# XuyangBai/PointDSC

Hardware: AMD Instinct MI355X
Metric: point-cloud pairs/sec @ N=5000 corr (higher is better)
Workload: dtype f32 (attention products as fp16x3 split (fp16 hi+lo operand pairs, three f16 MFMAs per product), f32 accumulate; fc_message / PointCN products as fp16 hi+lo split; spatial-consistency matrix stored as unorm16); 1 GPU; 3DMatch-like synthetic correspondences (BASELINE.json configs[2]): N=5000 corr, 32 pairs per step sharded over 1 GPU(s) = 32 per GPU, 12-layer PointDSC, seeded random weights; num_corr=5000, pairs_per_gpu=32, global_batch=32, compat_format=u16, layer_gemm=h3, att_leaves=canonical, latency_mode=False, range_guard=lazy (pipeline), collective=none (single process, no process group)

## Files before the change

include/pointdsc_hip.h:

```cpp
#ifndef POINTDSC_HIP_H
#define POINTDSC_HIP_H

#include <stddef.h>

#ifdef __cplusplus
extern "C" {
#endif

#define PDSC_VERSION 9
#define PDSC_CHANNELS 128
#define PDSC_MAX_K 64
#define PDSC_MAX_POWER_ITERS 32

enum pdsc_status {
    PDSC_OK = 0,
    PDSC_ERR_ARG = -1,
    PDSC_ERR_WORKSPACE = -2,
    PDSC_ERR_LAUNCH = -3
};

typedef struct pdsc_config {
    int in_dim;
    int num_layers;
    int num_channels;
// ... 128 lines not shown
size_t pdsc_wfrag_fold_head_bytes(void);
int pdsc_layer_prefers_block(int bs, int N);
int pdsc_layer_h3_uses_coop(int bs, int N);
size_t pdsc_wfrag_tail_bytes(void);
size_t pdsc_wfrag_head_bytes(void);
int pdsc_wfrag_build_tail(const float* w1, const float* b1, const float* w2, const float* b2, const float* w3,
                          const float* b3, void* out, int gemm_format, void* stream);
int pdsc_wfrag_build_head(const float* wp, const float* bp, const float* wq, const float* bq, void* out,
                          int gemm_format, void* stream);

size_t pdsc_attention_scratch_bytes(int bs, int N, int nsplit);
int    pdsc_attention_default_split(int bs, int N);
int    pdsc_sc_attention(const float* qkv, const float* compat, long long ld, float* msg,
                         void* scratch, size_t scratch_bytes, int bs, int N, int nsplit, void* stream);

size_t pdsc_split_q_bytes(int bs, int N);
size_t pdsc_split_kv_bytes(int bs, int N);
int    pdsc_pack_qkv_split(const float* qkv, void* q_split, void* kv_tiles, int bs, int N, void* stream);
size_t pdsc_attention_split_scratch_bytes(int bs, int N, int nsplit);
int    pdsc_attention_split_default_split(int bs, int N);
int    pdsc_attention_leaf_count(int N);
int    pdsc_attention_leaf_plan(int bs, int N, int leaves_mode, int* nsplit, int* nleaf);
size_t pdsc_attention_leaf_scratch_bytes(int bs, int N, int leaves_mode);
int    pdsc_sc_attention_split(const void* q_split, const void* kv_tiles, const float* compat, long long ld,
                               float* msg, void* scratch, size_t scratch_bytes, int bs, int N, int nsplit,
                               void* stream);
int    pdsc_sc_attention_split_u16(const void* q_split, const void* kv_tiles, const unsigned short* compat_u16, long long ld,
                                   float* msg, void* scratch, size_t scratch_bytes, int bs, int N, int nsplit,
                                   void* stream);

int pdsc_attention_trace(long long* device_buffer);

int pdsc_attention_leaf_split_override(int d);

int pdsc_layer_trace(long long* device_buffer);

int pdsc_classifier_hidden(const float* feat, const float* W1, const float* b1, const float* W2, const float* b2, float* h2,
                           int M, void* stream);

int pdsc_normalize_confidence(const float* feat, const float* h2, const float* w3, const float* b3,
                              float* normed, float* conf, int M, void* stream);

int pdsc_nms_keys(const float* src_keypts, const float* conf, float radius, float* keys,
                  int bs, int N, void* stream);
size_t pdsc_nms_workspace_bytes(int bs, int N);
int pdsc_nms_keys_grid(const float* src_keypts, const float* conf, float radius, float* keys, void* workspace,
                       size_t workspace_bytes, int bs, int N, void* stream);
int pdsc_rank_select(const float* keys, int* seeds, int bs, int N, int num_seeds, void* stream);

int pdsc_knn_seeds(const float* normed, const int* seeds, float* dist_scratch, int* knn_idx,
                   int bs, int N, int S, int k, void* stream);
int pdsc_knn_seeds_form(const float* normed, const float* normed_pf, const int* seeds, float* dist_scratch, int* knn_idx,
                        int bs, int N, int S, int k, int form, void* stream);
int pdsc_normalize_confidence_pf(const float* feat, const float* h2, const float* w3, const float* b3, float* normed,
                                 float* normed_pf, float* conf, int bs, int N, void* stream);

int pdsc_seed_power_iteration(const float* normed, const float* src_keypts, const float* tgt_keypts,
                              const int* knn_idx, const float* sigma, const float* sigma_spat,
                              float* eig_iters, unsigned int* conv_mask, float* seed_M,
                              int bs, int N, int S, int k, int num_iterations, void* stream);

int pdsc_seed_transforms(const float* src_keypts, const float* tgt_keypts, const int* knn_idx,
                         const float* eig_iters, const unsigned int* conv_mask, float* seed_trans,
                         float* seed_weights ,
                         int bs, int N, int S, int k, int num_iterations, void* stream);

int pdsc_seed_solve(const float* normed, const float* src_keypts, const float* tgt_keypts, const int* knn_idx,
                    const float* sigma, const float* sigma_spat, float* eig_iters, unsigned int* conv_mask, float* seed_M,
                    float* seed_trans, float* seed_weights, int bs, int N, int S, int k, int num_iterations, void* stream);

int pdsc_rigid_transform_3d(const float* A, const float* B, const float* weights, float weight_threshold,
                            float* T, int bs, int n, void* stream);

int pdsc_score_hypotheses(const float* seed_trans, const float* src_keypts, const float* tgt_keypts,
                          float inlier_threshold, int* counts, int bs, int N, int S, void* stream);
int pdsc_select_best(const int* counts, const float* seed_trans, const float* src_keypts,
                     const float* tgt_keypts, float inlier_threshold, int* best, float* initial_trans,
                     float* labels, int bs, int N, int S, void* stream);

int pdsc_post_refinement(const float* initial_trans, const float* src_keypts, const float* tgt_keypts,
                         float threshold, int max_iters, float* final_trans, int* solves,
                         int bs, int N, void* stream);

int pdsc_forward_testing(const pdsc_config* cfg, const float* wpack, const void* wsplit ,
                         const float* corr_pos, const float* src_keypts, const float* tgt_keypts,
                         int bs, int N, int num_seeds,
                         float* final_trans, float* final_labels,
                         void* workspace, size_t workspace_bytes, void* stream);

int pdsc_forward_testing_ragged(const pdsc_config* cfg, const float* wpack, const void* wsplit,
                                const float* corr_pos, const float* src_keypts, const float* tgt_keypts,
                                int bs, int N, int num_seeds, const int* num_corr, const int* num_seeds_per_pair, int n_min,
                                float* final_trans, float* final_labels,
                                void* workspace, size_t workspace_bytes, void* stream);

int pdsc_forward_testing_streams(const pdsc_config* cfg, const float* wpack, const void* wsplit,
                                 const float* corr_pos, const float* src_keypts, const float* tgt_keypts,
                                 int bs, int N, int num_seeds, const int* num_corr ,
                                 const int* num_seeds_per_pair, int n_min,
                                 float* final_trans, float* final_labels,
                                 void* workspace, size_t workspace_bytes,
                                 void* stream, void* tail_stream, void* fork_event, void* join_event);

int pdsc_forward_validation(const pdsc_config* cfg, const float* wpack, const void* wsplit,
                            const float* corr_pos, const float* src_keypts, const float* tgt_keypts,
                            int bs, int N, int num_seeds, float* final_trans, float* logits,
// ... 155 lines not shown
```

pointdsc_amd/_lib.py:

```python
from __future__ import annotations

import ctypes as C
import os
from pathlib import Path

PKG = Path(__file__).resolve().parent
LIB_PATH = Path(os.environ.get("POINTDSC_HIP_LIB", PKG / "libpointdsc_hip.so"))


class PointDSCLibraryError(RuntimeError):
    pass


class PdscConfig(C.Structure):
    _fields_ = [
        ("in_dim", C.c_int), ("num_layers", C.c_int), ("num_channels", C.c_int),
        ("num_iterations", C.c_int), ("k", C.c_int), ("refine_iters", C.c_int),
        ("inlier_threshold", C.c_float), ("nms_radius", C.c_float), ("refine_threshold", C.c_float),
        ("attention_precision", C.c_int), ("compat_format", C.c_int), ("layer_gemm", C.c_int),
        ("att_leaves", C.c_int), ("value_fold", C.c_int),
    ]


W_SECTIONS = [
# ... 16 lines not shown
SIGNATURES = {
    "pdsc_version": (_i, []),
    "pdsc_set_range_report": (_i, [_vp]),
    "pdsc_last_error": (C.c_char_p, []),
    "pdsc_experiments_enabled": (_i, []),
    "pdsc_wpack_floats": (_ll, [_cfgp]),
    "pdsc_wpack_offset": (_ll, [_cfgp, _i, _i]),
    "pdsc_compat_ld": (_ll, [_i]),
    "pdsc_workspace_bytes": (_sz, [_cfgp, _i, _i, _i]),
    "pdsc_workspace_offset": (_ll, [_cfgp, _i, _i, _i, C.c_char_p]),
    "pdsc_spatial_compat": (_i, [_vp, _vp, _vp, _vp, _vp, _ll, _i, _i, _vp]),
    "pdsc_spatial_compat_u16": (_i, [_vp, _vp, _vp, _vp, _ll, _i, _i, _vp]),
    "pdsc_selftest_exact_math": (_i, [_vp, _f, _vp, _vp, _ll, _vp]),
    "pdsc_selftest_mfma_valu_neighbour": (_i, [_vp, _i, _i, _vp]),
    "pdsc_classifier_hidden": (_i, [_vp, _vp, _vp, _vp, _vp, _vp, _i, _vp]),
    "pdsc_linear": (_i, [_vp, _ll, _vp, _vp, _vp, _ll, _vp, _ll, _i, _i, _i, _i, _vp]),
    "pdsc_layer0": (_i, [_vp, _i, _vp, _vp, _vp, _i, _vp]),
    "pdsc_layer_run": (_i, [C.POINTER(PdscLayerCall), _vp]),
    "pdsc_wsplit_bytes": (_sz, [_cfgp]),
    "pdsc_wsplit_offset": (_ll, [_cfgp, _i, _i]),
    "pdsc_wsplit_build": (_i, [_cfgp, _vp, _vp, _vp]),
    "pdsc_layer_prefers_block": (_i, [_i, _i]),
    "pdsc_layer_h3_uses_coop": (_i, [_i, _i]),
    "pdsc_wfrag_tail_bytes": (_sz, []),
    "pdsc_wfrag_head_bytes": (_sz, []),
    "pdsc_wfrag_fold_tail_bytes": (_sz, []),
    "pdsc_wfrag_fold_head_bytes": (_sz, []),
    "pdsc_wfrag_build_tail": (_i, [_vp] * 7 + [_i, _vp]),
    "pdsc_wfrag_build_head": (_i, [_vp] * 5 + [_i, _vp]),
    "pdsc_sc_attention_split_partials": (_i, [_vp, _vp, _vp, _i, _ll, _vp, _sz, _i, _i, _i, _i, _vp]),
    "pdsc_split_q_bytes": (_sz, [_i, _i]),
    "pdsc_split_kv_bytes": (_sz, [_i, _i]),
    "pdsc_pack_qkv_split": (_i, [_vp, _vp, _vp, _i, _i, _vp]),
    "pdsc_attention_split_scratch_bytes": (_sz, [_i, _i, _i]),
    "pdsc_attention_split_default_split": (_i, [_i, _i]),
    "pdsc_attention_leaf_count": (_i, [_i]),
    "pdsc_attention_leaf_plan": (_i, [_i, _i, _i, C.POINTER(C.c_int), C.POINTER(C.c_int)]),
    "pdsc_attention_leaf_scratch_bytes": (_sz, [_i, _i, _i]),
    "pdsc_attention_trace": (_i, [_vp]),
    "pdsc_attention_leaf_split_override": (_i, [_i]),
    "pdsc_layer_trace": (_i, [_vp]),
    "pdsc_sc_attention_split": (_i, [_vp, _vp, _vp, _ll, _vp, _vp, _sz, _i, _i, _i, _vp]),
    "pdsc_sc_attention_split_u16": (_i, [_vp, _vp, _vp, _ll, _vp, _vp, _sz, _i, _i, _i, _vp]),
    "pdsc_attention_scratch_bytes": (_sz, [_i, _i, _i]),
    "pdsc_attention_default_split": (_i, [_i, _i]),
    "pdsc_sc_attention": (_i, [_vp, _vp, _ll, _vp, _vp, _sz, _i, _i, _i, _vp]),
    "pdsc_normalize_confidence": (_i, [_vp, _vp, _vp, _vp, _vp, _vp, _i, _vp]),
    "pdsc_nms_keys": (_i, [_vp, _vp, _f, _vp, _i, _i, _vp]),
    "pdsc_nms_workspace_bytes": (_sz, [_i, _i]),
    "pdsc_nms_keys_grid": (_i, [_vp, _vp, _f, _vp, _vp, _sz, _i, _i, _vp]),
    "pdsc_rank_select": (_i, [_vp, _vp, _i, _i, _i, _vp]),
    "pdsc_knn_seeds": (_i, [_vp, _vp, _vp, _vp, _i, _i, _i, _i, _vp]),
    "pdsc_knn_seeds_form": (_i, [_vp, _vp, _vp, _vp, _vp, _i, _i, _i, _i, _i, _vp]),
    "pdsc_normalize_confidence_pf": (_i, [_vp, _vp, _vp, _vp, _vp, _vp, _vp, _i, _i, _vp]),
    "pdsc_seed_power_iteration": (_i, [_vp, _vp, _vp, _vp, _vp, _vp, _vp, _vp, _vp, _i, _i, _i, _i, _i, _vp]),
    "pdsc_seed_solve": (_i, [_vp] * 11 + [_i, _i, _i, _i, _i, _vp]),
    "pdsc_seed_transforms": (_i, [_vp, _vp, _vp, _vp, _vp, _vp, _vp, _i, _i, _i, _i, _i, _vp]),
    "pdsc_rigid_transform_3d": (_i, [_vp, _vp, _vp, _f, _vp, _i, _i, _vp]),
    "pdsc_score_hypotheses": (_i, [_vp, _vp, _vp, _f, _vp, _i, _i, _i, _vp]),
    "pdsc_select_best": (_i, [_vp, _vp, _vp, _vp, _f, _vp, _vp, _vp, _i, _i, _i, _vp]),
    "pdsc_post_refinement": (_i, [_vp, _vp, _vp, _f, _i, _vp, _vp, _i, _i, _vp]),
    "pdsc_profile_enable": (_i, [_i]),
    "pdsc_profile_reset": (_i, []),
    "pdsc_profile_set_stride": (_i, [_i, _i]),
    "pdsc_profile_read": (_i, [_i, C.POINTER(C.c_double), C.POINTER(C.c_int)]),
    "pdsc_match_scratch_bytes": (_sz, [_i, _i]),
    "pdsc_match_descriptors": (_i, [_vp, _vp, _i, _i, _i, _vp, _vp, _vp, _sz, _vp]),
    "pdsc_match_descriptors_ip": (_i, [_vp, _vp, _i, _i, _i, _vp, _vp, _vp, _sz, _vp]),
    "pdsc_select_correspondences": (_i, [_vp, _vp, _i, _vp, _vp, _vp]),
    "pdsc_build_corr_pos": (_i, [_vp, _vp, _vp, _vp, _vp, _vp, _vp, _vp]),
    "pdsc_sm_workspace_bytes": (_sz, [_i, _i]),
    "pdsc_sm_baseline": (_i, [_vp, _vp, _vp, _f, _i, _i, _vp, _vp, _vp, _vp, _sz, _i, _i, _vp]),
    "pdsc_sm_baseline_form": (_i, [_vp, _vp, _vp, _f, _i, _i, _vp, _vp, _vp, _vp, _sz, _i, _i, _i, _vp]),
    "pdsc_pmc_adjacency": (_i, [_vp, _f, _vp, _ll, _i, _i, _vp]),
    "pdsc_pmc_workspace_bytes": (_sz, [_i, _i]),
    "pdsc_pmc_baseline": (_i, [_vp, _vp, _vp, _f, _i, _vp, _vp, _vp, _vp, _vp, _sz, _i, _i, _vp]),
    "pdsc_pmc_baseline_ex": (_i, [_vp, _vp, _vp, _f, _i, _vp, _vp, _vp, _vp, _vp, _sz, _i, _i, _i, C.POINTER(C.c_float), _vp]),
    "pdsc_cal_confidence_workspace_bytes": (_sz, [_i, _i]),
    "pdsc_cal_confidence": (_i, [_vp, _ll, _vp, _i, _i, _vp, _vp, _sz, _i, _i, _vp]),
    "pdsc_eval_stats": (_i, [_vp, _vp, _vp, _vp, _f, _f, _vp, _i, _i, _vp]),
    "pdsc_loss_workspace_bytes": (_sz, [_i, _i]),
    "pdsc_classification_loss": (_i, [_vp, _vp, _vp, _i, _vp, _vp, _vp, _sz, _i, _i, _vp]),
    "pdsc_sm_loss_matrix": (_i, [_vp, _ll, _vp, _i, _vp, _vp, _vp, _sz, _i, _i, _vp]),
    "pdsc_sm_loss_features": (_i, [_vp, _vp, _vp, _i, _vp, _vp, _vp, _vp, _sz, _i, _i, _vp]),
    "pdsc_transformation_loss": (_i, [_vp, _vp, _vp, _vp, _vp, _f, _f, _vp, _vp, _sz, _i, _i, _vp]),
    "pdsc_sc_attention_lse": (_i, [_vp, _vp, _ll, _vp, _vp, _vp, _sz, _i, _i, _i, _vp]),
    "pdsc_attention_backward_workspace_bytes": (_sz, [_i, _i]),
    "pdsc_sc_attention_backward": (_i, [_vp, _vp, _ll, _vp, _vp, _vp, _vp, _vp, _sz, _i, _i, _vp]),
    "pdsc_attention_backward_default_split": (_i, [_i, _i]),
    "pdsc_attention_backward_split_workspace_bytes": (_sz, [_i, _i, _i]),
    "pdsc_sc_attention_backward_split": (_i, [_vp, _vp, _ll, _vp, _vp, _vp, _vp, _vp, _sz, _i, _i, _i, _vp]),
    "pdsc_feature_compat_backward_workspace_bytes": (_sz, [_i, _i]),
    "pdsc_feature_compat_backward": (_i, [_vp, _vp, _vp, _ll, _vp, _vp, _vp, _sz, _i, _i, _vp]),
    "pdsc_seed_solve_backward_workspace_bytes": (_sz, [_i, _i, _i, _i]),
    "pdsc_seed_solve_backward": (_i, [_vp] * 11 + [_sz, _i, _i, _i, _i, _i, _vp]),
    "pdsc_transformation_loss_grad": (_i, [_vp, _vp, _vp, _vp, _vp, _vp, _sz, _i, _i, _vp]),
    "pdsc_icp_workspace_bytes": (_sz, [_i, _i, _i]),
    "pdsc_icp_refine": (_i, [_vp, _vp, _vp, _vp, _vp, C.c_double, C.c_double, C.c_double, _i, _vp, _vp, _vp, _vp, _vp, _vp, _vp,
                             _sz, _i, _i, _i, _vp]),
    "pdsc_information_workspace_bytes": (_sz, [_i, _i, _i]),
    "pdsc_information_matrix": (_i, [_vp, _vp, _vp, _vp, _vp, C.c_double, _vp, _vp, _vp, _vp, _sz, _i, _i, _i, _vp]),
    "pdsc_voxel_keys": (_i, [_vp, _vp, C.c_double, _vp, _i, _i, _vp]),
    "pdsc_voxel_means": (_i, [_vp, _vp, _vp, _vp, _vp, _i, _i, _vp]),
    "pdsc_hybrid_neighbours_workspace_bytes": (_sz, [_i, _i]),
    "pdsc_hybrid_neighbours": (_i, [_vp, _vp, C.c_double, _i, _vp, _vp, _vp, _vp, _sz, _i, _i, _vp]),
    "pdsc_estimate_normals": (_i, [_vp, _vp, _vp, _vp, _i, C.POINTER(C.c_double), _vp, _i, _i, _vp]),
# ... 57 lines not shown
```

pointdsc_amd/csrc/seeds.hip:

```cpp
#include <math.h>
#include <stdlib.h>
#include "pdsc_common.h"
#include "ragged.h"

namespace pdsc {

int knn_dist_rows(const float* normed, const int* seeds, float* dist, long long ldd, int bs, int N, int S,
                  hipStream_t st);

__global__ __launch_bounds__(256) void normalize_conf_kernel(const float* __restrict__ feat, const float* __restrict__ h2,
                                                             const float* __restrict__ w3, const float* __restrict__ b3,
                                                             float* __restrict__ normed, float* __restrict__ conf, int M) {
    const int lane = threadIdx.x & 63;
    const long long row = (long long)blockIdx.x * 4 + (threadIdx.x >> 6);
    if (row >= M) return;
    const float2 v = *reinterpret_cast<const float2*>(feat + row * PDSC_CHANNELS + lane * 2);
    const float ss = wave_sum(fmaf(v.y, v.y, v.x * v.x));
    const float nrm = fmaxf(sqrtf(ss), 1e-12f);
    float2 o;
    o.x = v.x / nrm;
    o.y = v.y / nrm;
    *reinterpret_cast<float2*>(normed + row * PDSC_CHANNELS + lane * 2) = o;
    float p = lane < 32 ? h2[row * 32 + lane] * w3[lane] : 0.f;
    p = wave_sum(p);
// ... 464 lines not shown
        if (splits < min_splits) splits = min_splits;
        if (splits > N) splits = N;
        const int slice = pdsc::ceil_div(N, splits);
        splits = pdsc::ceil_div(N, slice);
        hipLaunchKernelGGL(pdsc::nms_flags_kernel, dim3(row_blocks, splits, bs), dim3(256), 0, st, src, conf, radius2, keys, N, slice);
        return pdsc::check_launch("pdsc_nms_keys");
    }
}

static float nms_radius2(float radius) { return pdsc::sqrt_threshold_radicand(radius); }

extern "C" size_t pdsc_nms_workspace_bytes(int bs, int N) {
    if (bs <= 0 || N <= 0) return 0;
    return (size_t)bs * pdsc::nms_ws_pair_bytes(N);
}

namespace pdsc {

int launch_nms_keys_grid(const float* src, const float* conf, float radius, float* keys, void* workspace, size_t workspace_bytes,
                         int bs, int N, const int* nvalid, hipStream_t st) {
    PDSC_REQUIRE(src && conf && keys, "pdsc_nms_keys_grid: null pointer");
    PDSC_REQUIRE(bs > 0 && N > 0, "pdsc_nms_keys_grid: bs=%d N=%d", bs, N);
    if (!(radius > 0.f) || !(radius < INFINITY) || !workspace) {
        PDSC_REQUIRE(!nvalid, "pdsc_nms_keys_grid: ragged batches need a positive finite nms_radius and the grid workspace");
        return pdsc_nms_keys(src, conf, radius, keys, bs, N, st);
    }
    if (workspace_bytes < pdsc_nms_workspace_bytes(bs, N)) {
        set_error("pdsc_nms_keys_grid: workspace %zu < %zu bytes", workspace_bytes, pdsc_nms_workspace_bytes(bs, N));
        return PDSC_ERR_WORKSPACE;
    }
    const size_t ws_pair = nms_ws_pair_bytes(N);
    hipLaunchKernelGGL(nms_grid_kernel, dim3(bs), dim3(1024), 0, st, src, conf, radius, (unsigned char*)workspace, ws_pair, N, nvalid);
    int rc = check_launch("pdsc_nms_keys_grid(grid)");
    if (rc != PDSC_OK) return rc;
    hipLaunchKernelGGL(nms_window_kernel, dim3(ceil_div(N, 256), bs), dim3(256), 0, st, (const unsigned char*)workspace, ws_pair,
                       nms_radius2(radius), keys, N, nvalid);
    return check_launch("pdsc_nms_keys_grid(window)");
}

int launch_rank_select(const float* keys, int* seeds, int bs, int N, int num_seeds, const int* nvalid, const int* svalid, hipStream_t st,
                       unsigned int* conv_mask_init) {
    PDSC_REQUIRE(keys && seeds, "pdsc_rank_select: null pointer");
    PDSC_REQUIRE(bs > 0 && N > 0 && num_seeds >= 0 && num_seeds <= N, "pdsc_rank_select: bs=%d N=%d S=%d", bs, N, num_seeds);
    if (num_seeds == 0) return conv_mask_init ? launch_fill_u32(conv_mask_init, 0xFFFFFFFFu, (size_t)bs, st) : PDSC_OK;
    const size_t lds_bytes = (size_t)num_seeds * sizeof(unsigned long long);
    PDSC_REQUIRE(lds_bytes <= 128 * 1024, "pdsc_rank_select: num_seeds=%d exceeds the single-workgroup LDS list (16384)", num_seeds);
    const int rc = ensure_dynamic_lds(reinterpret_cast<const void*>(&seed_select_kernel), lds_bytes > 65536 ? 128 * 1024 : 65536,
                                      "pdsc_rank_select(dynamic LDS)");
    if (rc != PDSC_OK) return rc;
    hipLaunchKernelGGL(seed_select_kernel, dim3(bs), dim3(SEL_THREADS), lds_bytes, st, keys, seeds, N, num_seeds, nvalid, svalid, conv_mask_init);
    return check_launch("pdsc_rank_select");
}

constexpr int KF_ROWS = 32, KF_CAP = 256, KF_KEEP = 96, KF_MAX_WANT = 48;

struct KnnFusedArgs {
    const float* X;
    const float* Xpf;
    const int* seeds;
    int* knn_idx;
    int NS, S, k, idx_bits;
    int bs, nrb;
    const int* nvalid;
};

__global__ __launch_bounds__(256, 2) void knn_fused_kernel(KnnFusedArgs a) {
    extern __shared__ __attribute__((aligned(16))) unsigned long long kf_dyn[];
    unsigned long long (*list)[KF_CAP] = reinterpret_cast<unsigned long long (*)[KF_CAP]>(kf_dyn);
    __shared__ float tau[KF_ROWS];
    __shared__ int cnt[KF_ROWS];
    __shared__ unsigned long long gmin[4][64];
    const int t = threadIdx.x, lane = t & 63, wave = t >> 6, l31 = lane & 31, h = lane >> 5;
    int b, rb;
    {
        const int nrb = a.nrb, L = blockIdx.x;
        if ((a.bs & 7) == 0) {
            const int xcd = L & 7, idx = L >> 3;
            b = xcd + 8 * (idx / nrb);
            rb = idx % nrb;
        } else {
            b = L / nrb;
            rb = L % nrb;
        }
    }
    const int r0 = rb * KF_ROWS;
    const int N = a.nvalid ? a.nvalid[b] : a.NS;
    const float* X = a.X + (size_t)b * a.NS * PDSC_CHANNELS;
    const int want = a.k + 1;
    const unsigned long long idx_mask = (1ULL << a.idx_bits) - 1ULL;
    if (t < KF_ROWS) { tau[t] = INFINITY; cnt[t] = 0; }

    f32x4 af[16];
    {
        const int row = a.seeds[(size_t)b * a.S + min(r0 + l31, a.S - 1)];
        const float* p = X + (size_t)row * PDSC_CHANNELS + 4 * h;
#pragma unroll
        for (int q = 0; q < 16; ++q) af[q] = *reinterpret_cast<const f32x4*>(p + 8 * q);
    }
    const int nblocks = (N + 31) >> 5, rounds = (nblocks + 3) >> 2;
    f32x4 bf[16];
    const int Npf = (a.NS + 31) & ~31;
    const float* Xpf = a.Xpf ? a.Xpf + (size_t)b * Npf * PDSC_CHANNELS + lane * 4 : nullptr;
    auto load_b = [&](int cb) {
        if (Xpf) {
            const float* p = Xpf + (size_t)min(cb, nblocks - 1) * 32 * PDSC_CHANNELS;
#pragma unroll
            for (int q = 0; q < 16; ++q) bf[q] = *reinterpret_cast<const f32x4*>(p + 256 * q);
        } else {
            const int col = min(cb * 32 + l31, N - 1);
            const float* p = X + (size_t)col * PDSC_CHANNELS + 4 * h;
#pragma unroll
            for (int q = 0; q < 16; ++q) bf[q] = *reinterpret_cast<const f32x4*>(p + 8 * q);
        }
    };
    load_b(wave);
    __syncthreads();
    for (int rd = 0; rd < rounds; ++rd) {
        const int cb = rd * 4 + wave;
        f32x16 acc;
#pragma unroll
        for (int r = 0; r < 16; ++r) acc[r] = 0.f;
#pragma unroll
        for (int q = 0; q < 16; ++q)
#pragma unroll
            for (int e = 0; e < 4; ++e) acc = __builtin_amdgcn_mfma_f32_32x32x2f32(af[q][e], bf[q][e], acc, 0, 0, 0);
        load_b(cb + 4);
        const int col = cb * 32 + l31;
        if (col < N) {
#pragma unroll
            for (int r = 0; r < 16; ++r) {
                const int row = (r & 3) + 8 * (r >> 2) + 4 * h;
                const float v = 2.0f - 2.0f * acc[r];
                if (v <= tau[row] && r0 + row < a.S) {
                    const unsigned long long key = ((unsigned long long)float_order_bits(v) << a.idx_bits) | (unsigned)col;
                    const int slot = atomicAdd(&cnt[row], 1);
                    list[row][slot] = key;
                }
            }
        }
        __syncthreads();
        for (int rr = 0; rr < 8; ++rr) {
            const int row = wave * 8 + rr;
            const int n = cnt[row];
            if (n <= KF_CAP - 128) continue;
            unsigned long long e[KF_CAP / 64], mine = ~0ULL;
#pragma unroll
            for (int u = 0; u < KF_CAP / 64; ++u) {
                e[u] = lane + 64 * u < n ? list[row][lane + 64 * u] : ~0ULL;
                mine = e[u] < mine ? e[u] : mine;
            }
            gmin[wave][lane] = mine;
            __builtin_amdgcn_fence(__ATOMIC_RELEASE, "wavefront");
            __builtin_amdgcn_wave_barrier();
            __builtin_amdgcn_fence(__ATOMIC_ACQUIRE, "wavefront");
            int rk = 0;
#pragma unroll 8
            for (int u = 0; u < 64; ++u) rk += gmin[wave][u] < mine;
            const unsigned long long vote = __ballot(rk == want - 1);
            const int src = __ffsll((long long)vote) - 1;
            unsigned long long ub = ((unsigned long long)(unsigned)__builtin_amdgcn_readlane((int)(mine >> 32), src) << 32) |
                                    (unsigned)__builtin_amdgcn_readlane((int)(mine & 0xffffffffULL), src);
            int kept = 0;
#pragma unroll
            for (int u = 0; u < KF_CAP / 64; ++u) {
                const bool keep = e[u] <= ub;
                const unsigned long long bal = __ballot(keep);
                if (keep) list[row][kept + __popcll(bal & ((1ULL << lane) - 1ULL))] = e[u];
                kept += __popcll(bal);
            }
            __builtin_amdgcn_fence(__ATOMIC_RELEASE, "wavefront");
            __builtin_amdgcn_wave_barrier();
            __builtin_amdgcn_fence(__ATOMIC_ACQUIRE, "wavefront");
            if (kept > KF_KEEP) {
                unsigned long long f[KF_CAP / 64], cand = 0ULL;
                int rank[KF_CAP / 64];
#pragma unroll
                for (int u = 0; u < KF_CAP / 64; ++u) { f[u] = lane + 64 * u < kept ? list[row][lane + 64 * u] : ~0ULL; rank[u] = 0; }
                for (int j = 0; j < kept; ++j) {
                    const unsigned long long o = list[row][j];
#pragma unroll
                    for (int u = 0; u < KF_CAP / 64; ++u) rank[u] += o < f[u];
                }
                __builtin_amdgcn_fence(__ATOMIC_RELEASE, "wavefront");
                __builtin_amdgcn_wave_barrier();
                __builtin_amdgcn_fence(__ATOMIC_ACQUIRE, "wavefront");
#pragma unroll
                for (int u = 0; u < KF_CAP / 64; ++u) {
                    const bool real = lane + 64 * u < kept;
                    if (real && rank[u] < want) list[row][rank[u]] = f[u];
                    if (real && rank[u] == want - 1) cand = f[u];
                }
                const unsigned long long who = __ballot(cand != 0ULL);
                const int sl = __ffsll((long long)who) - 1;
                ub = ((unsigned long long)(unsigned)__builtin_amdgcn_readlane((int)(cand >> 32), sl) << 32) |
                     (unsigned)__builtin_amdgcn_readlane((int)(cand & 0xffffffffULL), sl);
                kept = want;
            }
            if (lane == 0) {
                cnt[row] = kept;
                const unsigned int ob = (unsigned int)(ub >> a.idx_bits);
                tau[row] = __uint_as_float((ob & 0x80000000u) ? (ob & 0x7fffffffu) : ~ob);
            }
        }
        __syncthreads();
    }
    for (int rr = 0; rr < 8; ++rr) {
        const int row = wave * 8 + rr;
        if (r0 + row >= a.S) continue;
        const int n = cnt[row];
        unsigned long long f[KF_CAP / 64];
        int rank[KF_CAP / 64];
#pragma unroll
        for (int u = 0; u < KF_CAP / 64; ++u) { f[u] = lane + 64 * u < n ? list[row][lane + 64 * u] : ~0ULL; rank[u] = 0; }
        for (int j = 0; j < n; ++j) {
            const unsigned long long o = list[row][j];
#pragma unroll
            for (int u = 0; u < KF_CAP / 64; ++u) rank[u] += o < f[u];
        }
#pragma unroll
        for (int u = 0; u < KF_CAP / 64; ++u)
            if (lane + 64 * u < n && rank[u] >= 1 && rank[u] < want)
                a.knn_idx[((size_t)b * a.S + r0 + row) * a.k + (rank[u] - 1)] = (int)(f[u] & idx_mask);
    }
}

int launch_knn_seeds(const float* normed, const int* seeds, float* dist_scratch, int* knn_idx, int bs, int N, int S, int k,
                     const int* nvalid, hipStream_t st) {
    return launch_knn_seeds_form(normed, nullptr, seeds, dist_scratch, knn_idx, bs, N, S, k, nvalid, 0, st);
}

bool knn_seeds_uses_fused(int bs, int N, int S, int k) {
    return k + 1 <= KF_MAX_WANT && N >= 256 && (long long)bs * ceil_div(S, KF_ROWS) >= 384;
}

int launch_knn_seeds_form(const float* normed, const float* normed_pf, const int* seeds, float* dist_scratch, int* knn_idx, int bs, int N,
                          int S, int k, const int* nvalid, int form, hipStream_t st) {
    PDSC_REQUIRE(form >= 0 && form <= 2, "pdsc_knn_seeds: form=%d", form);
    const bool fits = k + 1 <= KF_MAX_WANT && N >= 256;
    PDSC_REQUIRE(form != 2 || fits, "pdsc_knn_seeds: the fused form needs k + 1 <= %d and N >= 256 (k=%d, N=%d)", KF_MAX_WANT, k, N);
    if (form == 2 || (form == 0 && knn_seeds_uses_fused(bs, N, S, k))) {
        PDSC_REQUIRE(normed && seeds && knn_idx, "pdsc_knn_seeds: null pointer");
        PDSC_REQUIRE(bs > 0 && N > 1 && S > 0, "pdsc_knn_seeds: bs=%d N=%d S=%d", bs, N, S);
        PDSC_REQUIRE(k >= 1 && k <= PDSC_MAX_K && k <= N - 1, "pdsc_knn_seeds: k=%d (N=%d, max %d)", k, N, PDSC_MAX_K);
        KnnFusedArgs a{};
        a.X = normed; a.Xpf = normed_pf; a.seeds = seeds; a.knn_idx = knn_idx; a.NS = N; a.S = S; a.k = k; a.nvalid = nvalid;
        a.idx_bits = 1;
        while ((1 << a.idx_bits) < N) ++a.idx_bits;
        const size_t lds_bytes = (size_t)KF_ROWS * KF_CAP * sizeof(unsigned long long);
        const int rc_lds = ensure_dynamic_lds(reinterpret_cast<const void*>(&knn_fused_kernel), lds_bytes, "pdsc_knn_seeds(fused, dynamic LDS)");
        if (rc_lds != PDSC_OK) return rc_lds;
        a.bs = bs; a.nrb = ceil_div(S, KF_ROWS);
        hipLaunchKernelGGL(knn_fused_kernel, dim3((unsigned)(a.nrb * bs)), dim3(256), lds_bytes, st, a);
        return check_launch("pdsc_knn_seeds(fused)");
    }

    PDSC_REQUIRE(normed && seeds && dist_scratch && knn_idx, "pdsc_knn_seeds: null pointer");
    PDSC_REQUIRE(bs > 0 && N > 1 && S > 0, "pdsc_knn_seeds: bs=%d N=%d S=%d", bs, N, S);
    PDSC_REQUIRE(k >= 1 && k <= PDSC_MAX_K && k <= N - 1, "pdsc_knn_seeds: k=%d (N=%d, max %d)", k, N, PDSC_MAX_K);
    PDSC_REQUIRE((size_t)N * 4 <= 144 * 1024, "pdsc_knn_seeds: N=%d exceeds the single-workgroup LDS row (36864)", N);
    const long long ldd = pdsc_compat_ld(N);
    int rc = knn_dist_rows(normed, seeds, dist_scratch, ldd, bs, N, S, st);
    if (rc != PDSC_OK) return rc;
    int idx_bits = 1;
    while ((1 << idx_bits) < N) ++idx_bits;
    const size_t lds_bytes = (size_t)N * sizeof(unsigned int);
    {
        const int rc_lds = ensure_dynamic_lds(reinterpret_cast<const void*>(&knn_select_kernel), 144 * 1024, "pdsc_knn_seeds(dynamic LDS)");
        if (rc_lds != PDSC_OK) return rc_lds;
    }
    hipLaunchKernelGGL(knn_select_kernel, dim3(S, bs), dim3(KNN_THREADS), lds_bytes, st, dist_scratch, ldd, knn_idx, N, S, k, idx_bits, nvalid);
    return check_launch("pdsc_knn_seeds");
}

}

extern "C" int pdsc_nms_keys_grid(const float* src, const float* conf, float radius, float* keys, void* workspace,
                                  size_t workspace_bytes, int bs, int N, void* stream) {
    return pdsc::launch_nms_keys_grid(src, conf, radius, keys, workspace, workspace_bytes, bs, N, nullptr, (hipStream_t)stream);
}

extern "C" int pdsc_rank_select(const float* keys, int* seeds, int bs, int N, int num_seeds, void* stream) {
    return pdsc::launch_rank_select(keys, seeds, bs, N, num_seeds, nullptr, nullptr, (hipStream_t)stream);
}

extern "C" int pdsc_knn_seeds_form(const float* normed, const float* normed_pf, const int* seeds, float* dist_scratch, int* knn_idx,
                                   int bs, int N, int S, int k, int form, void* stream) {
    return pdsc::launch_knn_seeds_form(normed, normed_pf, seeds, dist_scratch, knn_idx, bs, N, S, k, nullptr, form, (hipStream_t)stream);
}

extern "C" int pdsc_normalize_confidence_pf(const float* feat, const float* h2, const float* w3, const float* b3, float* normed,
                                            float* normed_pf, float* conf, int bs, int N, void* stream) {
    return pdsc::launch_normalize_conf_pf(feat, h2, w3, b3, normed, normed_pf, conf, bs, N, (hipStream_t)stream);
}

extern "C" int pdsc_knn_seeds(const float* normed, const int* seeds, float* dist_scratch, int* knn_idx, int bs, int N,
                              int S, int k, void* stream) {
    return pdsc::launch_knn_seeds(normed, seeds, dist_scratch, knn_idx, bs, N, S, k, nullptr, (hipStream_t)stream);
}
```

Measured before the change: 2541 pairs/s.

## Restructure fused kNN with LDS ring staging, per-wave lists, and column split

Rewrites the fused seed kNN kernel. Column blocks are now staged into a three-slot LDS ring via global_load_lds, so all four waves share each block and the next loads overlap compute. Each wave owns its own seed-row group and keeps wave-private candidate lists with ballot-based appends instead of LDS atomics. List trimming now uses a pivot-based selection and is interleaved with the MFMA chain of the next block. When there are too few workgroups to fill the GPU, columns are split across workgroups, with a merge kernel that combines partial top-k lists held in dist_scratch. This adds a second launch and extra scratch traffic in the split case, and smaller lists may trigger trims more often.

New measurement: 2459 pairs/s. 0.968x the previous value.

```diff
diff --git a/include/pointdsc_hip.h b/include/pointdsc_hip.h
--- a/include/pointdsc_hip.h
+++ b/include/pointdsc_hip.h
@@ -204,6 +204,9 @@
                    int bs, int N, int S, int k, void* stream);
 int pdsc_knn_seeds_form(const float* normed, const float* normed_pf, const int* seeds, float* dist_scratch, int* knn_idx,
                         int bs, int N, int S, int k, int form, void* stream);
+int pdsc_knn_seeds_form_ragged(const float* normed, const float* normed_pf, const int* seeds, float* dist_scratch, int* knn_idx,
+                               int bs, int N, int S, int k, const int* nvalid, int form, void* stream);
+int pdsc_knn_fused_split_override(int c);
 int pdsc_normalize_confidence_pf(const float* feat, const float* h2, const float* w3, const float* b3, float* normed,
                                  float* normed_pf, float* conf, int bs, int N, void* stream);
 
diff --git a/pointdsc_amd/_lib.py b/pointdsc_amd/_lib.py
--- a/pointdsc_amd/_lib.py
+++ b/pointdsc_amd/_lib.py
@@ -92,6 +92,8 @@
     "pdsc_rank_select": (_i, [_vp, _vp, _i, _i, _i, _vp]),
     "pdsc_knn_seeds": (_i, [_vp, _vp, _vp, _vp, _i, _i, _i, _i, _vp]),
     "pdsc_knn_seeds_form": (_i, [_vp, _vp, _vp, _vp, _vp, _i, _i, _i, _i, _i, _vp]),
+    "pdsc_knn_seeds_form_ragged": (_i, [_vp, _vp, _vp, _vp, _vp, _i, _i, _i, _i, _vp, _i, _vp]),
+    "pdsc_knn_fused_split_override": (_i, [_i]),
     "pdsc_normalize_confidence_pf": (_i, [_vp, _vp, _vp, _vp, _vp, _vp, _vp, _i, _i, _vp]),
     "pdsc_seed_power_iteration": (_i, [_vp, _vp, _vp, _vp, _vp, _vp, _vp, _vp, _vp, _i, _i, _i, _i, _i, _vp]),
     "pdsc_seed_solve": (_i, [_vp] * 11 + [_i, _i, _i, _i, _i, _vp]),
diff --git a/pointdsc_amd/csrc/seeds.hip b/pointdsc_amd/csrc/seeds.hip
--- a/pointdsc_amd/csrc/seeds.hip
+++ b/pointdsc_amd/csrc/seeds.hip
@@ -540,43 +540,161 @@
     return check_launch("pdsc_rank_select");
 }
 
-constexpr int KF_ROWS = 32, KF_CAP = 256, KF_KEEP = 96, KF_MAX_WANT = 48;
+constexpr int KF_ROWS = 32, KF_WAVES = 4, KF_CAP = 104, KF_TRIM = KF_CAP - 32, KF_PER_LANE = (KF_CAP + 63) / 64, KF_MAX_WANT = 48;
+constexpr int KF_RING = 3, KF_BLOCK_BYTES = 32 * PDSC_CHANNELS * 4, KF_MAX_SPLIT = 32, KF_CUS = 256;
+constexpr int KF_OFF_LIST = KF_RING * KF_BLOCK_BYTES, KF_OFF_GMIN = KF_OFF_LIST + KF_WAVES * KF_ROWS * KF_CAP * 8,
+              KF_OFF_TAU = KF_OFF_GMIN + KF_WAVES * 64 * 8, KF_OFF_CNT = KF_OFF_TAU + KF_WAVES * KF_ROWS * 4,
+              KF_LDS_BYTES = KF_OFF_CNT + KF_WAVES * KF_ROWS * 4;
+static_assert(KF_TRIM >= 64 && KF_MAX_WANT <= 64 && KF_LDS_BYTES <= 160 * 1024, "fused kNN: list capacity / LDS budget");
+
+typedef __attribute__((address_space(1))) const void* kf_gptr_t;
+typedef __attribute__((address_space(3))) void* kf_lptr_t;
 
 struct KnnFusedArgs {
     const float* X;
     const float* Xpf;
     const int* seeds;
     int* knn_idx;
+    unsigned long long* scratch;
+    long long ldd;
     int NS, S, k, idx_bits;
-    int bs, nrb;
+    int bs, nrb, ngroups;
+    int csplit;
     const int* nvalid;
 };
 
-__global__ __launch_bounds__(256, 2) void knn_fused_kernel(KnnFusedArgs a) {
-    extern __shared__ __attribute__((aligned(16))) unsigned long long kf_dyn[];
-    unsigned long long (*list)[KF_CAP] = reinterpret_cast<unsigned long long (*)[KF_CAP]>(kf_dyn);
-    __shared__ float tau[KF_ROWS];
-    __shared__ int cnt[KF_ROWS];
-    __shared__ unsigned long long gmin[4][64];
+__device__ __forceinline__ void kf_wave_sync() {
+    __builtin_amdgcn_fence(__ATOMIC_RELEASE, "wavefront");
+    __builtin_amdgcn_wave_barrier();
+    __builtin_amdgcn_fence(__ATOMIC_ACQUIRE, "wavefront");
+}
+
+__device__ __forceinline__ unsigned long long kf_readlane64(unsigned long long v, int src) {
+    return ((unsigned long long)(unsigned)__builtin_amdgcn_readlane((int)(v >> 32), src) << 32) |
+           (unsigned)__builtin_amdgcn_readlane((int)(v & 0xffffffffULL), src);
+}
+
+constexpr int KF_PIVOTS = 24;
+__device__ __forceinline__ void kf_trim_row(unsigned long long* lrow, unsigned long long* gm, int want, int idx_bits, int lane,
+                                            float* tau_slot, int* cnt_slot) {
+    const int n = __builtin_amdgcn_readfirstlane(*cnt_slot);
+    unsigned long long e[KF_PER_LANE];
+#pragma unroll
+    for (int u = 0; u < KF_PER_LANE; ++u) e[u] = lane + 64 * u < n ? lrow[lane + 64 * u] : ~0ULL;
+    const int win = min(KF_TRIM, want + 8);
+    static_assert(KF_PER_LANE == 2, "kf_trim_row: two entries per lane");
+    unsigned long long in0 = n >= 64 ? ~0ULL : (1ULL << n) - 1ULL, in1 = n > 64 ? (1ULL << (n - 64)) - 1ULL : 0ULL, ub = 0ULL;
+    int kept = 0;
+    bool found = false;
+    for (int step = 0; step < KF_PIVOTS && (in0 | in1); ++step) {
+        const unsigned long long pivot = in1 ? kf_readlane64(e[1], __ffsll((long long)in1) - 1) : kf_readlane64(e[0], __ffsll((long long)in0) - 1);
+        const unsigned long long le0 = __ballot(e[0] <= pivot), le1 = __ballot(e[1] <= pivot);
+        const int c = __popcll(le0) + __popcll(le1);
+        if (c < want) { in0 &= ~le0; in1 &= ~le1; }
+        else if (c > win) {
+            if (in1) in1 &= in1 - 1; else in0 &= in0 - 1;
+            in0 &= le0; in1 &= le1;
+        } else { found = true; ub = pivot; break; }
+    }
+    if (!found) {
+        unsigned long long mine = ~0ULL;
+#pragma unroll
+        for (int u = 0; u < KF_PER_LANE; ++u) mine = e[u] < mine ? e[u] : mine;
+        gm[lane] = mine;
+        kf_wave_sync();
+        int rk = 0;
+#pragma unroll 8
+        for (int u = 0; u < 64; ++u) rk += gm[u] < mine;
+        const unsigned long long vote = __ballot(rk == want - 1);
+        ub = kf_readlane64(mine, __ffsll((long long)vote) - 1);
+    }
+#pragma unroll
+    for (int u = 0; u < KF_PER_LANE; ++u) {
+        const bool keep = e[u] <= ub;
+        const unsigned long long bal = __ballot(keep);
+        if (keep) lrow[kept + __popcll(bal & ((1ULL << lane) - 1ULL))] = e[u];
+        kept += __popcll(bal);
+    }
+    if (!found) {
+        kf_wave_sync();
+        if (kept > 64) {
+            unsigned long long f[KF_PER_LANE], cand = 0ULL;
+            int rank[KF_PER_LANE];
+#pragma unroll
+            for (int u = 0; u < KF_PER_LANE; ++u) { f[u] = lane + 64 * u < kept ? lrow[lane + 64 * u] : ~0ULL; rank[u] = 0; }
+            for (int j = 0; j < kept; ++j) {
+                const unsigned long long o = lrow[j];
+#pragma unroll
+                for (int u = 0; u < KF_PER_LANE; ++u) rank[u] += o < f[u];
+            }
+            kf_wave_sync();
+#pragma unroll
+            for (int u = 0; u < KF_PER_LANE; ++u) {
+                const bool real = lane + 64 * u < kept;
+                if (real && rank[u] < want) lrow[rank[u]] = f[u];
+                if (real && rank[u] == want - 1) cand = f[u];
+            }
+            const unsigned long long who = __ballot(cand != 0ULL);
+            ub = kf_readlane64(cand, __ffsll((long long)who) - 1);
+            kept = want;
+        }
+    }
+    if (lane == 0) {
+        *cnt_slot = kept;
+        const unsigned int ob = (unsigned int)(ub >> idx_bits);
+        *tau_slot = __uint_as_float((ob & 0x80000000u) ? (ob & 0x7fffffffu) : ~ob);
+    }
+    kf_wave_sync();
+}
+
+__device__ __forceinline__ void kf_rank_row(unsigned long long* lrow, int n, int lane, unsigned long long& f, int& rank) {
+    const int n8 = (n + 7) & ~7;
+    if (lane >= n && lane < n8) lrow[lane] = ~0ULL;
+    kf_wave_sync();
+    f = lane < n ? lrow[lane] : ~0ULL;
+    rank = 0;
+    for (int j = 0; j < n8; j += 8) {
+        unsigned long long o[8];
+#pragma unroll
+        for (int jj = 0; jj < 8; ++jj) o[jj] = lrow[j + jj];
+#pragma unroll
+        for (int jj = 0; jj < 8; ++jj) rank += o[jj] < f;
+    }
+}
+
+__global__ __launch_bounds__(256) void knn_fused_kernel(KnnFusedArgs a) {
+    extern __shared__ __attribute__((aligned(16))) unsigned char kf_lds[];
     const int t = threadIdx.x, lane = t & 63, wave = t >> 6, l31 = lane & 31, h = lane >> 5;
-    int b, rb;
+    unsigned long long* list = reinterpret_cast<unsigned long long*>(kf_lds + KF_OFF_LIST) + wave * KF_ROWS * KF_CAP;
+    unsigned long long* gmin = reinterpret_cast<unsigned long long*>(kf_lds + KF_OFF_GMIN) + wave * 64;
+    float* tau = reinterpret_cast<float*>(kf_lds + KF_OFF_TAU) + wave * KF_ROWS;
+    int* cnt = reinterpret_cast<int*>(kf_lds + KF_OFF_CNT) + wave * KF_ROWS;
+    int b, g, c;
     {
-        const int nrb = a.nrb, L = blockIdx.x;
+        const int per = a.ngroups * a.csplit, L = blockIdx.x;
+        int within;
         if ((a.bs & 7) == 0) {
             const int xcd = L & 7, idx = L >> 3;
-            b = xcd + 8 * (idx / nrb);
-            rb = idx % nrb;
+            b = xcd + 8 * (idx / per);
+            within = idx % per;
         } else {
-            b = L / nrb;
-            rb = L % nrb;
-        }
-    }
-    const int r0 = rb * KF_ROWS;
+            b = L / per;
+            within = L % per;
+        }
+        g = within / a.csplit;
+        c = within % a.csplit;
+    }
+    const int sb = g * KF_WAVES + wave, r0 = sb * KF_ROWS;
+    const bool owner = sb < a.nrb;
+    const int rows_valid = a.S - r0;
     const int N = a.nvalid ? a.nvalid[b] : a.NS;
     const float* X = a.X + (size_t)b * a.NS * PDSC_CHANNELS;
     const int want = a.k + 1;
     const unsigned long long idx_mask = (1ULL << a.idx_bits) - 1ULL;
-    if (t < KF_ROWS) { tau[t] = INFINITY; cnt[t] = 0; }
+    const int nblocks = (N + 31) >> 5;
+    const int cb0 = (int)((long long)c * nblocks / a.csplit), nb = (int)((long long)(c + 1) * nblocks / a.csplit) - cb0;
+    if (lane < KF_ROWS) { tau[lane] = INFINITY; cnt[lane] = 0; }
+    kf_wave_sync();
 
     f32x4 af[16];
     {
@@ -585,132 +703,173 @@
 #pragma unroll
         for (int q = 0; q < 16; ++q) af[q] = *reinterpret_cast<const f32x4*>(p + 8 * q);
     }
-    const int nblocks = (N + 31) >> 5, rounds = (nblocks + 3) >> 2;
-    f32x4 bf[16];
+    asm volatile("s_waitcnt vmcnt(0)" ::: "memory");
+
     const int Npf = (a.NS + 31) & ~31;
-    const float* Xpf = a.Xpf ? a.Xpf + (size_t)b * Npf * PDSC_CHANNELS + lane * 4 : nullptr;
-    auto load_b = [&](int cb) {
+    const float* Xpf = a.Xpf ? a.Xpf + (size_t)b * Npf * PDSC_CHANNELS + wave * 1024 + lane * 4 : nullptr;
+    auto stage = [&](int i, int slot) {
+        const int cb = cb0 + min(i, nb - 1);
+        unsigned char* dst = kf_lds + slot * KF_BLOCK_BYTES + wave * 4096;
         if (Xpf) {
-            const float* p = Xpf + (size_t)min(cb, nblocks - 1) * 32 * PDSC_CHANNELS;
-#pragma unroll
-            for (int q = 0; q < 16; ++q) bf[q] = *reinterpret_cast<const f32x4*>(p + 256 * q);
+            const float* p = Xpf + (size_t)cb * 32 * PDSC_CHANNELS;
+#pragma unroll
+            for (int u = 0; u < 4; ++u) __builtin_amdgcn_global_load_lds((kf_gptr_t)(p + 256 * u), (kf_lptr_t)(dst + 1024 * u), 16, 0, 0);
         } else {
-            const int col = min(cb * 32 + l31, N - 1);
-            const float* p = X + (size_t)col * PDSC_CHANNELS + 4 * h;
-#pragma unroll
-            for (int q = 0; q < 16; ++q) bf[q] = *reinterpret_cast<const f32x4*>(p + 8 * q);
+            const float* p = X + (size_t)min(cb * 32 + l31, N - 1) * PDSC_CHANNELS + 4 * h + 32 * wave;
+#pragma unroll
+            for (int u = 0; u < 4; ++u) __builtin_amdgcn_global_load_lds((kf_gptr_t)(p + 8 * u), (kf_lptr_t)(dst + 1024 * u), 16, 0, 0);
         }
     };
-    load_b(wave);
-    __syncthreads();
-    for (int rd = 0; rd < rounds; ++rd) {
-        const int cb = rd * 4 + wave;
-        f32x16 acc;
-#pragma unroll
-        for (int r = 0; r < 16; ++r) acc[r] = 0.f;
-#pragma unroll
-        for (int q = 0; q < 16; ++q)
-#pragma unroll
-            for (int e = 0; e < 4; ++e) acc = __builtin_amdgcn_mfma_f32_32x32x2f32(af[q][e], bf[q][e], acc, 0, 0, 0);
-        load_b(cb + 4);
-        const int col = cb * 32 + l31;
-        if (col < N) {
+
+    if (nb > 0) {
+        stage(0, 0);
+        stage(1, 1);
+        float tau_r[16];
+        int cnt_r[16];
+        unsigned int row_ok = 0;
+#pragma unroll
+        for (int r = 0; r < 16; ++r) {
+            tau_r[r] = INFINITY;
+            cnt_r[r] = 0;
+            row_ok |= ((r & 3) + 8 * (r >> 2) + 4 * h < rows_valid ? 1u : 0u) << r;
+        }
+        f32x16 old;
+        int old_col = 0;
+        unsigned int need = 0;
+        bool trimmed = false;
+        int slot = 0;
+        auto trim_one = [&]() {
+            const int row = __ffs((int)need) - 1;
+            need &= need - 1;
+            kf_trim_row(list + row * KF_CAP, gmin, want, a.idx_bits, lane, tau + row, cnt + row);
+            trimmed = true;
+        };
+        auto reload = [&]() {
+            if (trimmed) {
+#pragma unroll
+                for (int r = 0; r < 16; ++r) {
+                    const int row = (r & 3) + 8 * (r >> 2) + 4 * h;
+                    tau_r[r] = tau[row];
+                    cnt_r[r] = cnt[row];
+                }
+                trimmed = false;
+            }
+        };
+        auto file = [&](int r, bool col_ok) {
+            const float v = 2.0f - 2.0f * old[r];
+            const bool pass = col_ok && ((row_ok >> r) & 1u) && v <= tau_r[r];
+            const unsigned long long bal = __ballot(pass);
+            if (bal) {
+                const unsigned int half = h ? (unsigned int)(bal >> 32) : (unsigned int)bal;
+                const int row = (r & 3) + 8 * (r >> 2) + 4 * h;
+                if (pass)
+                    list[row * KF_CAP + cnt_r[r] + __popc(half & ((1u << l31) - 1u))] =
+                        ((unsigned long long)float_order_bits(v) << a.idx_bits) | (unsigned)old_col;
+                cnt_r[r] += __popc(half);
+            }
+        };
+        auto filed = [&]() {
+            unsigned int over = 0;
 #pragma unroll
             for (int r = 0; r < 16; ++r) {
                 const int row = (r & 3) + 8 * (r >> 2) + 4 * h;
-                const float v = 2.0f - 2.0f * acc[r];
-                if (v <= tau[row] && r0 + row < a.S) {
-                    const unsigned long long key = ((unsigned long long)float_order_bits(v) << a.idx_bits) | (unsigned)col;
-                    const int slot = atomicAdd(&cnt[row], 1);
-                    list[row][slot] = key;
+                if (l31 == 0) cnt[row] = cnt_r[r];
+                over |= (cnt_r[r] > KF_TRIM ? 1u : 0u) << row;
+            }
+            kf_wave_sync();
+            need = (unsigned int)__builtin_amdgcn_readlane((int)over, 0) | (unsigned int)__builtin_amdgcn_readlane((int)over, 32);
+        };
+        for (int i = 0; i < nb; ++i) {
+            asm volatile("s_waitcnt vmcnt(4) lgkmcnt(0)" ::: "memory");
+            __builtin_amdgcn_s_barrier();
+            asm volatile("" ::: "memory");
+            stage(i + 2, slot == 0 ? 2 : slot - 1);
+            if (owner) {
+                f32x4 bf[16];
+                const float* bp = reinterpret_cast<const float*>(kf_lds + slot * KF_BLOCK_BYTES) + lane * 4;
+#pragma unroll
+                for (int q = 0; q < 16; ++q) bf[q] = *reinterpret_cast<const f32x4*>(bp + 256 * q);
+                f32x16 acc;
+#pragma unroll
+                for (int r = 0; r < 16; ++r) acc[r] = 0.f;
+                const bool col_ok = old_col < N;
+#pragma unroll
+                for (int q = 0; q < 16; ++q) {
+                    acc = __builtin_amdgcn_mfma_f32_32x32x2f32(af[q][0], bf[q][0], acc, 0, 0, 0);
+                    if (q == 0) {
+                        while (need) trim_one();
+                        reload();
+                    }
+                    acc = __builtin_amdgcn_mfma_f32_32x32x2f32(af[q][1], bf[q][1], acc, 0, 0, 0);
+                    if (i > 0) file(q, col_ok);
+                    acc = __builtin_amdgcn_mfma_f32_32x32x2f32(af[q][2], bf[q][2], acc, 0, 0, 0);
+                    acc = __builtin_amdgcn_mfma_f32_32x32x2f32(af[q][3], bf[q][3], acc, 0, 0, 0);
                 }
-            }
-        }
-        __syncthreads();
-        for (int rr = 0; rr < 8; ++rr) {
-            const int row = wave * 8 + rr;
-            const int n = cnt[row];
-            if (n <= KF_CAP - 128) continue;
-            unsigned long long e[KF_CAP / 64], mine = ~0ULL;
-#pragma unroll
-            for (int u = 0; u < KF_CAP / 64; ++u) {
-                e[u] = lane + 64 * u < n ? list[row][lane + 64 * u] : ~0ULL;
-                mine = e[u] < mine ? e[u] : mine;
-            }
-            gmin[wave][lane] = mine;
-            __builtin_amdgcn_fence(__ATOMIC_RELEASE, "wavefront");
-            __builtin_amdgcn_wave_barrier();
-            __builtin_amdgcn_fence(__ATOMIC_ACQUIRE, "wavefront");
-            int rk = 0;
-#pragma unroll 8
-            for (int u = 0; u < 64; ++u) rk += gmin[wave][u] < mine;
-            const unsigned long long vote = __ballot(rk == want - 1);
-            const int src = __ffsll((long long)vote) - 1;
-            unsigned long long ub = ((unsigned long long)(unsigned)__builtin_amdgcn_readlane((int)(mine >> 32), src) << 32) |
-                                    (unsigned)__builtin_amdgcn_readlane((int)(mine & 0xffffffffULL), src);
-            int kept = 0;
-#pragma unroll
-            for (int u = 0; u < KF_CAP / 64; ++u) {
-                const bool keep = e[u] <= ub;
-                const unsigned long long bal = __ballot(keep);
-                if (keep) list[row][kept + __popcll(bal & ((1ULL << lane) - 1ULL))] = e[u];
-                kept += __popcll(bal);
-            }
-            __builtin_amdgcn_fence(__ATOMIC_RELEASE, "wavefront");
-            __builtin_amdgcn_wave_barrier();
-            __builtin_amdgcn_fence(__ATOMIC_ACQUIRE, "wavefront");
-            if (kept > KF_KEEP) {
-                unsigned long long f[KF_CAP / 64], cand = 0ULL;
-                int rank[KF_CAP / 64];
-#pragma unroll
-                for (int u = 0; u < KF_CAP / 64; ++u) { f[u] = lane + 64 * u < kept ? list[row][lane + 64 * u] : ~0ULL; rank[u] = 0; }
-                for (int j = 0; j < kept; ++j) {
-                    const unsigned long long o = list[row][j];
-#pragma unroll
-                    for (int u = 0; u < KF_CAP / 64; ++u) rank[u] += o < f[u];
-                }
-                __builtin_amdgcn_fence(__ATOMIC_RELEASE, "wavefront");
-                __builtin_amdgcn_wave_barrier();
-                __builtin_amdgcn_fence(__ATOMIC_ACQUIRE, "wavefront");
-#pragma unroll
-                for (int u = 0; u < KF_CAP / 64; ++u) {
-                    const bool real = lane + 64 * u < kept;
-                    if (real && rank[u] < want) list[row][rank[u]] = f[u];
-                    if (real && rank[u] == want - 1) cand = f[u];
-                }
-                const unsigned long long who = __ballot(cand != 0ULL);
-                const int sl = __ffsll((long long)who) - 1;
-                ub = ((unsigned long long)(unsigned)__builtin_amdgcn_readlane((int)(cand >> 32), sl) << 32) |
-                     (unsigned)__builtin_amdgcn_readlane((int)(cand & 0xffffffffULL), sl);
-                kept = want;
-            }
-            if (lane == 0) {
-                cnt[row] = kept;
-                const unsigned int ob = (unsigned int)(ub >> a.idx_bits);
-                tau[row] = __uint_as_float((ob & 0x80000000u) ? (ob & 0x7fffffffu) : ~ob);
-            }
-        }
-        __syncthreads();
-    }
-    for (int rr = 0; rr < 8; ++rr) {
-        const int row = wave * 8 + rr;
-        if (r0 + row >= a.S) continue;
-        const int n = cnt[row];
-        unsigned long long f[KF_CAP / 64];
-        int rank[KF_CAP / 64];
-#pragma unroll
-        for (int u = 0; u < KF_CAP / 64; ++u) { f[u] = lane + 64 * u < n ? list[row][lane + 64 * u] : ~0ULL; rank[u] = 0; }
-        for (int j = 0; j < n; ++j) {
-            const unsigned long long o = list[row][j];
-#pragma unroll
-            for (int u = 0; u < KF_CAP / 64; ++u) rank[u] += o < f[u];
-        }
-#pragma unroll
-        for (int u = 0; u < KF_CAP / 64; ++u)
-            if (lane + 64 * u < n && rank[u] >= 1 && rank[u] < want)
-                a.knn_idx[((size_t)b * a.S + r0 + row) * a.k + (rank[u] - 1)] = (int)(f[u] & idx_mask);
-    }
-}
+                if (i > 0) filed();
+                old = acc;
+                old_col = (cb0 + i) * 32 + l31;
+            }
+            slot = slot == 2 ? 0 : slot + 1;
+        }
+        asm volatile("s_waitcnt vmcnt(0)" ::: "memory");
+        if (owner) {
+            while (need) trim_one();
+            reload();
+            const bool col_ok = old_col < N;
+#pragma unroll
+            for (int r = 0; r < 16; ++r) file(r, col_ok);
+            filed();
+        }
+    }
+    if (!owner) return;
+
+    for (int row = 0; row < KF_ROWS; ++row) {
+        if (row >= rows_valid) break;
+        if (__builtin_amdgcn_readfirstlane(cnt[row]) > 64) kf_trim_row(list + row * KF_CAP, gmin, want, a.idx_bits, lane, tau + row, cnt + row);
+        const int n = __builtin_amdgcn_readfirstlane(cnt[row]);
+        unsigned long long f;
+        int rank;
+        kf_rank_row(list + row * KF_CAP, n, lane, f, rank);
+        const size_t seed = (size_t)b * a.S + r0 + row;
+        if (a.csplit == 1) {
+            if (lane < n && rank >= 1 && rank < want) a.knn_idx[seed * a.k + (rank - 1)] = (int)(f & idx_mask);
+        } else {
+            unsigned long long* out = a.scratch + seed * (size_t)(a.ldd / 2) + (size_t)c * want;
+            if (lane < n && rank < want) out[rank] = f;
+            if (lane >= n && lane < want) out[lane] = ~0ULL;
+        }
+    }
+}
+
+__global__ __launch_bounds__(256) void knn_fused_merge_kernel(const unsigned long long* __restrict__ scratch, long long ldd,
+                                                              int* __restrict__ knn_idx, long long seeds_total, int k, int idx_bits,
+                                                              int csplit) {
+    extern __shared__ __attribute__((aligned(16))) unsigned long long kf_merge_lds[];
+    const int lane = threadIdx.x & 63, wave = threadIdx.x >> 6;
+    const long long seed = (long long)blockIdx.x * 4 + wave;
+    if (seed >= seeds_total) return;
+    const int want = k + 1, M = csplit * want, M8 = (M + 7) & ~7;
+    const unsigned long long* src = scratch + seed * (ldd / 2);
+    unsigned long long* all = kf_merge_lds + wave * M8;
+    for (int i = lane; i < M8; i += 64) all[i] = i < M ? src[i] : ~0ULL;
+    kf_wave_sync();
+    const unsigned long long idx_mask = (1ULL << idx_bits) - 1ULL;
+    for (int i0 = 0; i0 < M; i0 += 128) {
+        const unsigned long long m0 = i0 + lane < M ? all[i0 + lane] : ~0ULL, m1 = i0 + 64 + lane < M ? all[i0 + 64 + lane] : ~0ULL;
+        int rank0 = 0, rank1 = 0;
+        for (int j = 0; j < M8; j += 8) {
+            unsigned long long o[8];
+#pragma unroll
+            for (int jj = 0; jj < 8; ++jj) o[jj] = all[j + jj];
+#pragma unroll
+            for (int jj = 0; jj < 8; ++jj) { rank0 += o[jj] < m0; rank1 += o[jj] < m1; }
+        }
+        if (m0 != ~0ULL && rank0 >= 1 && rank0 < want) knn_idx[seed * k + (rank0 - 1)] = (int)(m0 & idx_mask);
+        if (m1 != ~0ULL && rank1 >= 1 && rank1 < want) knn_idx[seed * k + (rank1 - 1)] = (int)(m1 & idx_mask);
+    }
+}
+
+static int g_knn_fused_split_override = 0;
 
 int launch_knn_seeds(const float* normed, const int* seeds, float* dist_scratch, int* knn_idx, int bs, int N, int S, int k,
                      const int* nvalid, hipStream_t st) {
@@ -734,12 +893,35 @@
         a.X = normed; a.Xpf = normed_pf; a.seeds = seeds; a.knn_idx = knn_idx; a.NS = N; a.S = S; a.k = k; a.nvalid = nvalid;
         a.idx_bits = 1;
         while ((1 << a.idx_bits) < N) ++a.idx_bits;
-        const size_t lds_bytes = (size_t)KF_ROWS * KF_CAP * sizeof(unsigned long long);
-        const int rc_lds = ensure_dynamic_lds(reinterpret_cast<const void*>(&knn_fused_kernel), lds_bytes, "pdsc_knn_seeds(fused, dynamic LDS)");
+        a.bs = bs; a.nrb = ceil_div(S, KF_ROWS); a.ngroups = ceil_div(a.nrb, KF_WAVES);
+        const int want = k + 1;
+        const long long ldd = pdsc_compat_ld(N);
+        const long long fit = ldd * 4 / ((long long)want * 8);
+        int csplit = g_knn_fused_split_override;
+        if (csplit > 0) {
+            PDSC_REQUIRE(csplit == 1 || dist_scratch, "pdsc_knn_seeds: the fused form with a column split of %d needs dist_scratch", csplit);
+            PDSC_REQUIRE(csplit == 1 || csplit <= fit,
+                         "pdsc_knn_seeds: a column split of %d needs %lld bytes of dist_scratch per seed, a row holds %lld (k=%d, N=%d)", csplit,
+                         (long long)csplit * want * 8, ldd * 4, k, N);
+        } else {
+            const long long wgs = (long long)bs * a.ngroups;
+            long long cs = wgs >= KF_CUS ? 1 : KF_CUS / wgs;
+            cs = std::min(cs, (long long)std::max(1, ceil_div(N, 32) / 8));
+            cs = std::min(cs, std::min(fit, (long long)KF_MAX_SPLIT));
+            csplit = dist_scratch && cs > 1 ? (int)cs : 1;
+        }
+        PDSC_REQUIRE(csplit == 1 || ((uintptr_t)dist_scratch & 7) == 0, "pdsc_knn_seeds: dist_scratch must be 8-byte aligned");
+        a.csplit = csplit; a.ldd = ldd; a.scratch = reinterpret_cast<unsigned long long*>(dist_scratch);
+        const int rc_lds = ensure_dynamic_lds(reinterpret_cast<const void*>(&knn_fused_kernel), KF_LDS_BYTES, "pdsc_knn_seeds(fused, dynamic LDS)");
         if (rc_lds != PDSC_OK) return rc_lds;
-        a.bs = bs; a.nrb = ceil_div(S, KF_ROWS);
-        hipLaunchKernelGGL(knn_fused_kernel, dim3((unsigned)(a.nrb * bs)), dim3(256), lds_bytes, st, a);
-        return check_launch("pdsc_knn_seeds(fused)");
+        hipLaunchKernelGGL(knn_fused_kernel, dim3((unsigned)(a.ngroups * csplit * bs)), dim3(256), KF_LDS_BYTES, st, a);
+        const int rc = check_launch("pdsc_knn_seeds(fused)");
+        if (rc != PDSC_OK || csplit == 1) return rc;
+        const long long seeds_total = (long long)bs * S;
+        hipLaunchKernelGGL(knn_fused_merge_kernel, dim3((unsigned)((seeds_total + 3) / 4)), dim3(256),
+                           (size_t)4 * ((csplit * want + 7) & ~7) * sizeof(unsigned long long), st, a.scratch, ldd, knn_idx,
+                           seeds_total, k, a.idx_bits, csplit);
+        return check_launch("pdsc_knn_seeds(fused, merge)");
     }
 
     PDSC_REQUIRE(normed && seeds && dist_scratch && knn_idx, "pdsc_knn_seeds: null pointer");
@@ -776,6 +958,18 @@
     return pdsc::launch_knn_seeds_form(normed, normed_pf, seeds, dist_scratch, knn_idx, bs, N, S, k, nullptr, form, (hipStream_t)stream);
 }
 
+extern "C" int pdsc_knn_seeds_form_ragged(const float* normed, const float* normed_pf, const int* seeds, float* dist_scratch, int* knn_idx,
+                                          int bs, int N, int S, int k, const int* nvalid, int form, void* stream) {
+    return pdsc::launch_knn_seeds_form(normed, normed_pf, seeds, dist_scratch, knn_idx, bs, N, S, k, nvalid, form, (hipStream_t)stream);
+}
+
+extern "C" int pdsc_knn_fused_split_override(int c) {
+    PDSC_REQUIRE(c >= 0 && c <= pdsc::KF_MAX_SPLIT, "pdsc_knn_fused_split_override: c=%d (0 = the launcher decides, else 1 .. %d column ranges)", c,
+                 pdsc::KF_MAX_SPLIT);
+    pdsc::g_knn_fused_split_override = c;
+    return PDSC_OK;
+}
+
 extern "C" int pdsc_normalize_confidence_pf(const float* feat, const float* h2, const float* w3, const float* b3, float* normed,
                                             float* normed_pf, float* conf, int bs, int N, void* stream) {
     return pdsc::launch_normalize_conf_pf(feat, h2, w3, b3, normed, normed_pf, conf, bs, N, (hipStream_t)stream);
```
